# mbway/turbo

Measured on AMD Instinct MI355X. Metric: acquisition evals/sec (M candidates, N training) + GP-fit ms, higher is better.
Workload: dtype f32

## Files before the change

### turbo_amd/_lib.py

```python
import ctypes
import importlib.util
import os
import sys

import numpy as np

_HERE = os.path.dirname(os.path.abspath(__file__))

os.environ.setdefault("GPU_MAX_HW_QUEUES", "8")
LIB_PATH = os.environ.get("TGP_LIBRARY") or os.path.join(_HERE, "csrc", "libturbogp.so")

OK, NOT_PD, BAD_ARG, HIP_ERROR, NOT_FITTED, NO_MEMORY, NO_DEVICE = 0, 1, 2, 3, 4, 5, 6
DEVICE_HOST = -1
F64, F32, F32X3, F32H2 = 0, 1, 2, 3
KERNELS = {"rbf": 0, "matern12": 1, "matern32": 2, "matern52": 3}
ACQ_NONE, ACQ_UCB, ACQ_PI, ACQ_EI, ACQ_SIGMA, ACQ_MES = 0, 1, 2, 3, 4, 5
BUF_K, BUF_L, BUF_LINV, BUF_ALPHA = 0, 1, 2, 3
BATCH_KB, BATCH_CL = 0, 1

SYMBOLS = (
    "tgp_create", "tgp_destroy", "tgp_last_error", "tgp_version", "tgp_fit", "tgp_fit_grad", "tgp_loo", "tgp_fit_loo_grad", "tgp_fit_optimise", "tgp_fit_lbfgsb", "tgp_set_private_stream",
    "tgp_set_overlap", "tgp_tuning", "tgp_mt19937_uniform_columns", "tgp_set_candidates_mt19937", "tgp_stream_status", "tgp_workers_acquire", "tgp_workers_release",
    "tgp_fit_append", "tgp_export_state", "tgp_import_state", "tgp_export_factor_dev", "tgp_import_factor_dev", "tgp_debug_read",
    "tgp_set_candidates", "tgp_set_candidates_dev", "tgp_gen_candidates", "tgp_gen_candidates_lhs", "tgp_lhs_design",
# ... 829 lines not shown
        assert Xq.ndim == 2 and Xq.shape[1] == self.D, "points must be (m, %d)" % self.D
        val = np.empty(Xq.shape[0])
        grad = np.empty(Xq.shape)
        self._check(self.lib.tgp_acq_grad(self._h, _ptr(Xq), Xq.shape[0], acq, float(sf), float(incumbent),
                                          float(param), _ptr(val), _ptr(grad)))
        return val, grad

    def profile_enable(self, on=True):
        self._check(self.lib.tgp_profile_enable(self._h, 1 if on else 0))

    def profile_reset(self):
        self._check(self.lib.tgp_profile_reset(self._h))

    def profile_read(self):
        tl, kl = ctypes.c_int64(), ctypes.c_int64()
        tm, km, fm, sm = (ctypes.c_double() for _ in range(4))
        self._check(self.lib.tgp_profile_read(self._h, ctypes.byref(tl), ctypes.byref(tm),
                                              ctypes.byref(kl), ctypes.byref(km),
                                              ctypes.byref(fm), ctypes.byref(sm)))
        return dict(trmm_launches=tl.value, trmm_ms=tm.value, kstar_launches=kl.value,
                    kstar_ms=km.value, last_fit_ms=fm.value, last_sweep_ms=sm.value)

    def last_timings(self):
        v = np.zeros(12)
        self._check(self.lib.tgp_last_timings(self._h, _ptr(v), 12))
        return dict(fit_ms=v[0], sweep_ms=v[1], grad_kinv_ms=v[2], grad_pairwise_ms=v[3], grad_ard_ms=v[4],
                    trmm_flops=v[5], sweep_f64=int(v[6]), small_fit_phases_us=[float(x) for x in v[7:12]])

    def last_prune(self):
        v = np.zeros(19)
        self._check(self.lib.tgp_last_timings(self._h, _ptr(v), 19))
        return dict(state=int(v[12]), lb_set=int(v[13]), survivors=int(v[14]), screen=int(v[16]), screen_arith=int(v[18]))

    def sweep_geometry(self):
        ch, npad = ctypes.c_int64(), ctypes.c_int64()
        self._check(self.lib.tgp_sweep_geometry(self._h, ctypes.byref(ch), ctypes.byref(npad)))
        return ch.value, npad.value
```

### turbo_amd/csrc/sweep_pruned.hpp

```cpp
#pragma once

namespace tgp {

struct BoundArgs {
    const double *mupart, *abspart; long ldpart; int njs;
    long m;
    double err_scale;
    const double *err;
    const double *wcoef;
    const double *wadd;
    double y_mean, y_std;
    double sig_lo, sig_hi;
    int acq; double sf, incumbent, param, margin;
    double *ub;
};

__global__ __launch_bounds__(256) void prune_bound_kernel(BoundArgs b) {
    const long c = (long)blockIdx.x * 256 + threadIdx.x;
    if (c >= b.m) return;
    double mun = 0.0, s = 0.0;
    for (int j = 0; j < b.njs; ++j) {
        mun += b.mupart[(long)j * b.ldpart + c];
        if (!b.err || b.wcoef) s += b.abspart[(long)j * b.ldpart + c];
    }
    double e = b.err ? b.err[c] : b.err_scale * s;
    if (b.wcoef) e = screen_h2_error(e, b.wcoef[c], s, b.wadd[0]);
    const double mu = b.y_std * (b.sf > 0.0 ? mun + e : mun - e) + b.y_mean;
    const double a_lo = acq_value(b.acq, b.sf, b.incumbent, b.param, mu, b.sig_lo);
    const double a_hi = acq_value(b.acq, b.sf, b.incumbent, b.param, mu, b.sig_hi);
    double a = a_lo > a_hi ? a_lo : a_hi;
    double scale = fabs(a);
    if (b.acq == TGP_ACQ_UCB) scale += fabs(mu) + fabs(b.param) * b.sig_hi;
    a += b.margin * scale;
    b.ub[c] = (isnan(a_lo) || isnan(a_hi) || isnan(a)) ? INFINITY : a;
}

__global__ __launch_bounds__(256) void prune_pick_kernel(const double *__restrict__ ub, long m, long gs,
                                                         long long *__restrict__ pick) {
    __shared__ double sv[256];
    __shared__ long long si[256];
    const long g0 = (long)blockIdx.x * gs;
    const long g1 = g0 + gs < m ? g0 + gs : m;
    Best b;
    for (long c = g0 + threadIdx.x; c < g1; c += 256) {
        const double u = ub[c];
        if (u > b.v) { b.v = u; b.i = c; }
    }
    b = block_argmax<256>(b, sv, si);
    if (threadIdx.x == 0) pick[blockIdx.x] = b.i == IDX_NONE ? g0 : b.i;
}

template <typename T>
__global__ __launch_bounds__(256) void prune_gather_kernel(const T *__restrict__ Cs, int Dp, const long long *__restrict__ idx,
                                                           long n, long rows, T *__restrict__ out) {
    const long total = rows * Dp;
    for (long i = (long)blockIdx.x * 256 + threadIdx.x; i < total; i += (long)gridDim.x * 256) {
        const long r = i / Dp;
        const int d = (int)(i - r * Dp);
        out[i] = r < n ? Cs[idx[r] * Dp + d] : (T)0;
    }
}

struct SurvArgs {
    const double *ub; long m;
    const long long *pick; long gs;
    const double *lb; double margin;
    int *bcnt; const int *boff;
    long long *sidx;
    const long long *src;
};

__device__ __forceinline__ bool prune_survives(const SurvArgs &s, long c) {
    const double lb = s.lb[0];
    const double bar = isinf(lb) ? lb : lb - s.margin * fabs(lb);
    return c < s.m && s.ub[c] >= bar && (s.src || s.pick[c / s.gs] != c);
}

__global__ __launch_bounds__(256) void prune_count_kernel(SurvArgs s) {
    __shared__ int wsum[4];
    const long c = (long)blockIdx.x * 256 + threadIdx.x;
    const unsigned long long bal = __ballot(prune_survives(s, c));
    if ((threadIdx.x & 63) == 0) wsum[threadIdx.x >> 6] = __popcll(bal);
    __syncthreads();
    if (threadIdx.x == 0) s.bcnt[blockIdx.x] = wsum[0] + wsum[1] + wsum[2] + wsum[3];
}

__global__ __launch_bounds__(1024) void prune_scan_kernel(const int *__restrict__ bcnt, int nb, int *__restrict__ boff,
                                                          long long *__restrict__ total) {
    __shared__ int part[1024];
    const int per = (nb + 1023) / 1024;
    const int b0 = (int)threadIdx.x * per;
    const int b1 = b0 + per < nb ? b0 + per : nb;
    int s = 0;
    for (int b = b0; b < b1; ++b) s += bcnt[b];
    part[threadIdx.x] = s;
    __syncthreads();
    for (int o = 1; o < 1024; o <<= 1) {
        const int v = (int)threadIdx.x >= o ? part[threadIdx.x - o] : 0;
        __syncthreads();
        part[threadIdx.x] += v;
        __syncthreads();
    }
    int run = part[threadIdx.x] - s;
    for (int b = b0; b < b1; ++b) { boff[b] = run; run += bcnt[b]; }
    if (threadIdx.x == 1023) total[0] = part[1023];
}

__global__ __launch_bounds__(256) void prune_scatter_kernel(SurvArgs s) {
    __shared__ int wsum[4];
    const long c = (long)blockIdx.x * 256 + threadIdx.x;
    const bool keep = prune_survives(s, c);
    const unsigned long long bal = __ballot(keep);
    const int lane = threadIdx.x & 63, w = threadIdx.x >> 6;
    if (lane == 0) wsum[w] = __popcll(bal);
    __syncthreads();
    int off = s.boff[blockIdx.x];
    for (int k = 0; k < w; ++k) off += wsum[k];
    if (keep) s.sidx[off + __popcll(bal & ((1ull << lane) - 1ull))] = s.src ? s.src[c] : c;
}

struct PruneWs {
    double *ub; long long *pick, *sidx, *misc; int *bcnt, *boff; void *cs;
    double *err, *ub1; long long *sidx1; float *nx;
    double *wcoef; unsigned char *xh; float *nxp, *absa; long ncap;
};
static size_t al256(size_t b) { return (b + 255) & ~(size_t)255; }

struct Carver {
    char *base = nullptr;
    size_t off = 0;
    template <typename U>
    U *take(size_t count, bool wanted = true) {
        U *ptr = base ? reinterpret_cast<U *>(base + off) : nullptr;
        if (wanted) off += al256(count * sizeof(U));
        return ptr;
    }
};

template <typename T>
static void prune_carve(const Context &c, int64_t npick, int64_t rows_cap, bool screen, bool h2, Carver &k, PruneWs &w) {
    const size_t M = (size_t)c.M, nb = (size_t)((c.M + 255) / 256), Mpad = (size_t)c.ws_Mpad;
    w.ncap = (long)((c.N + SCR_T - 1) / SCR_T + 1) * SCR_T;
    const size_t ncap = (size_t)w.ncap, nch = (size_t)((c.Dp + SCR_DC - 1) / SCR_DC);
    w.ub = k.take<double>(M);
    w.pick = k.take<long long>((size_t)npick);
    w.sidx = k.take<long long>(M);
    w.misc = k.take<long long>(32);
    w.bcnt = k.take<int>(nb);
    w.boff = k.take<int>(nb);
    w.cs = k.take<T>((size_t)rows_cap * c.Dp);
    w.err = k.take<double>(Mpad, screen);
    w.ub1 = k.take<double>((size_t)rows_cap, screen);
    w.sidx1 = k.take<long long>(M, screen);
    w.nx = k.take<float>((size_t)c.Np, screen);
    w.wcoef = k.take<double>(Mpad, h2);
    w.xh = k.take<unsigned char>(nch * ncap * 128, h2);
    w.nxp = k.take<float>(ncap, h2);
    w.absa = k.take<float>(ncap, h2);
}

template <typename T>
static hipError_t prune_workspace(Context &c, int64_t npick, int64_t rows_cap, bool screen, bool h2, PruneWs &w) {
    Carver count;
    prune_carve<T>(c, npick, rows_cap, screen, h2, count, w);
    TGP_TRY(c.d_prune.reserve(count.off, [&] { return hipStreamSynchronize(c.stream); }));
    Carver k{c.d_prune};
    prune_carve<T>(c, npick, rows_cap, screen, h2, k, w);
    return hipSuccess;
}

template <typename T>
static TrmmVariant contract_variant(const SweepPlan<T> &p, int64_t rows, int ntm) {
    TrmmVariant v;
    v.kern = p.early.kern; v.lds = trmm_glds_lds_bytes(); v.tile_m = 128; v.tile_n = 128; v.threads = 256;
    if ((rows / 128) * ntm >= CONTRACT_MIN_WGS) return v;
    if ((rows / 64) * ntm >= CONTRACT_MIN_WGS) {
        v.kern = trmm_sumsq_glds_narrow_kernel<T, 64>; v.lds = trmm_narrow_lds_bytes<64>(); v.tile_n = 64;
    } else {
        v.kern = trmm_sumsq_glds_narrow_kernel<T, 32>; v.lds = trmm_narrow_lds_bytes<32>(); v.tile_n = 32;
    }
    return v;
}

template <typename T>
static hipError_t contract_rows(Context &c, const SweepPlan<T> &p, const T *cs, int64_t n, ProfCursor &cur) {
    for (int64_t off = 0; off < n; off += c.launch_rows) {
        const int64_t m = n - off < c.launch_rows ? n - off : c.launch_rows;
        const int64_t rows = pad128(m);
        const int ntile = (int)c.Np / 128;
        const int njs_s = grid_splits(rows / (16 * kstar_ar(sizeof(T))), GATHER_KS_MIN_WGS, ntile, ntile);
        const int njs_g = njs_s > p.njs ? njs_s : p.njs;
        TGP_TRY(launch_kstar<T>(c, Kstar::SlabNoMean, cs + off * c.Dp, rows, njs_g, c.d_Ks[0].get(), c.d_mupart + off,
                                (long)c.Np / 16, 1.f, cur.st));
        cur.seg(1);
        TGP_TRY(launch_trmm<T>(c, p, contract_variant<T>(p, rows, p.n128), 0, off, rows, 0, p.n128, 0, true, cur.st));
        cur.seg(0, (double)m * (double)c.N * (double)c.N);
    }
    return hipSuccess;
}

enum class PruneGo { NotEligible, GatedOff, Go };
template <typename T>
static PruneGo prune_eligible(const Context &c, const SweepPlan<T> &p, const SweepCall &call) {
    const int acq = call.acq;
    if (call.mu || call.sigma || call.acqv) return PruneGo::NotEligible;
    if (acq != TGP_ACQ_EI && acq != TGP_ACQ_PI && acq != TGP_ACQ_UCB) return PruneGo::NotEligible;
    if (c.dtype != TGP_F32 && c.dtype != TGP_F64) return PruneGo::NotEligible;
    if (!p.mean_in_trmm || tuning_sweep_prune_now() == 0) return PruneGo::NotEligible;
    if (!(c.M > tuning().prune_top)) return PruneGo::NotEligible;
    if (!((double)c.M * (double)c.N * (double)c.N >= tuning_prune_min_work_now())) return PruneGo::NotEligible;
    const double u = sizeof(T) == 4 ? 0x1p-24 : 0x1p-53;
    const bool gate = c.noise > 0.0 && c.noise / (c.constant + c.noise) >= tuning().prune_tau * u;
    return gate ? PruneGo::Go : PruneGo::GatedOff;
}

template <typename T>
struct PruneRun {
    Context &c;
    const SweepPlan<T> &p;
    const SweepCall &call;
    PruneWs w;
    BoundArgs b;
    const T *Cs, *Xs;
    T *cs;
    int64_t gs, npick, keep;
    bool screen, h2;
    ProfCursor cur;
};

template <typename T>
static hipError_t tight_bound(PruneRun<T> &r, const T *rowsrc, int64_t rows, int64_t m, double *ub) {
    Context &c = r.c;
    const int njs_b = grid_splits(rows / (16 * kstar_ar(sizeof(T))), BOUND_MIN_WGS, r.p.njs, r.p.njs);
    TGP_TRY(launch_kstar<T>(c, Kstar::Bound, rowsrc, rows, njs_b, c.d_part.get(), c.d_mupart, 0L, 1.f, c.stream));
    r.cur.seg(1);
    r.b.njs = njs_b; r.b.m = m; r.b.err = nullptr; r.b.wcoef = nullptr; r.b.ub = ub;
    hipLaunchKernelGGL(prune_bound_kernel, dim3((unsigned)((m + 255) / 256)), dim3(256), 0, c.stream, r.b);
    return hipGetLastError();
}

static hipError_t screen_h2_bound(PruneRun<float> &r, int64_t xb, int njs_s) {
    Context &c = r.c;
    const PruneWs &w = r.w;
    const int N = (int)c.N, Dp = (int)c.Dp;
    const ScreenH2Terms et = screen_h2_error_terms(c.constant, (int)c.D, N);
    ScreenH2Scal *scal = reinterpret_cast<ScreenH2Scal *>(w.misc + 8);
    static_assert(sizeof(ScreenH2Scal) <= 256 - 64, "the scalars live behind misc's first eight words");
    ScreenH2PrepArgs a{};
    a.Xs = r.Xs; a.alpha = c.d_alpha; a.N = N; a.Dp = Dp; a.nch = (Dp + SCR_DC - 1) / SCR_DC; a.ncap = w.ncap;
    a.P = et.P; a.Qc = et.Qc; a.Qw = et.Qw;
    a.Xh = w.xh; a.nxp = w.nxp; a.absa = w.absa; a.scal = scal;
    hipLaunchKernelGGL(screen_h2_prep_kernel, dim3((unsigned)((N + 255) / 256)), dim3(256), 0, c.stream, a);
    TGP_TRY(hipGetLastError());
    r.cur.restart();
    ScreenH2Args g{};
    g.Cs = r.Cs; g.Xh = w.xh; g.nxp = w.nxp; g.absa = w.absa; g.scal = scal;
    g.mupart = c.d_mupart; g.wpart = c.d_part; g.err = w.err; g.wcoef = w.wcoef; g.ldpart = c.ws_Mpad; g.ncap = w.ncap;
    g.Dp = Dp; g.constant = c.constant; g.dcoef = et.dcoef;
    hipLaunchKernelGGL(prune_screen_h2_kernel, dim3((unsigned)xb, (unsigned)njs_s), dim3(256), 0, c.stream, g);
    TGP_TRY(hipGetLastError());
// ... 11 lines not shown
    double *scal = reinterpret_cast<double *>(w.misc + 8);
    hipLaunchKernelGGL(screen_stats_kernel, dim3(1), dim3(1024), 0, c.stream, r.Xs, c.d_alpha, N, (int)c.Np, Dp, et.P, et.Q, w.nx, scal);
    TGP_TRY(hipGetLastError());
    r.cur.restart();
    ScreenArgs g{};
    g.Cs = r.Cs; g.Xs = r.Xs; g.alpha = c.d_alpha; g.nx = w.nx; g.scal = scal;
    g.mupart = c.d_mupart; g.err = w.err; g.ldpart = c.ws_Mpad;
    g.N = N; g.Np = (int)c.Np; g.Dp = Dp; g.constant = c.constant;
    hipLaunchKernelGGL(prune_screen_kernel, dim3((unsigned)xb, (unsigned)njs_s), dim3(256), 0, c.stream, g);
    TGP_TRY(hipGetLastError());
    r.cur.seg(2);
    c.prune_arith = 1;
    r.b.wcoef = nullptr;
    return hipSuccess;
}

template <typename T>
static hipError_t bound_all(PruneRun<T> &r) {
    Context &c = r.c;
    if (!r.screen) return tight_bound<T>(r, r.Cs, c.ws_Mpad, c.M, r.w.ub);
    if constexpr (sizeof(T) == 4) {
        const int64_t xb = c.ws_Mpad / SCR_T;
        const int njt = ((int)c.N + SCR_T - 1) / SCR_T;
        const int njs_s = grid_splits(xb, SCREEN_MIN_WGS, r.p.njs, njt < r.p.njs ? njt : r.p.njs);
        TGP_TRY(r.h2 ? screen_h2_bound(r, xb, njs_s) : screen_f32_bound(r, xb, njs_s));
        r.b.njs = njs_s; r.b.m = c.M; r.b.err = r.w.err; r.b.ub = r.w.ub;
        hipLaunchKernelGGL(prune_bound_kernel, dim3((unsigned)((c.M + 255) / 256)), dim3(256), 0, c.stream, r.b);
        return hipGetLastError();
    }
    return hipSuccess;
}

template <typename T>
static hipError_t gather_rows(PruneRun<T> &r, const long long *idx, int64_t n) {
    const int Dp = (int)r.c.Dp;
    const long total = (long)pad128(n) * Dp;
    const long blocks = (total + 255) / 256 < 8192 ? (total + 255) / 256 : 8192;
    hipLaunchKernelGGL(prune_gather_kernel<T>, dim3((unsigned)blocks), dim3(256), 0, r.c.stream, r.Cs, Dp, idx, (long)n,
                       (long)pad128(n), r.cs);
    return hipGetLastError();
}

template <typename T>
static hipError_t finalize_rows(PruneRun<T> &r, const long long *idx, int64_t n, int64_t blk0) {
    FinArgs f = fin_args<T>(r.c, r.p, r.call);
    f.base_pairs = r.p.nunits;
    f.njs = 1;
    f.off = blk0 * FIN_BLOCK; f.m = n;
    f.gidx = idx;
    hipLaunchKernelGGL(finalize_kernel, dim3((unsigned)((n + FIN_BLOCK - 1) / FIN_BLOCK)), dim3(FIN_BLOCK), 0, r.c.stream, f);
    return hipGetLastError();
}

template <typename T>
static hipError_t lb_set(PruneRun<T> &r, int64_t &nblk) {
    Context &c = r.c;
    hipLaunchKernelGGL(prune_pick_kernel, dim3((unsigned)r.npick), dim3(256), 0, c.stream, r.w.ub, (long)c.M, (long)r.gs, r.w.pick);
    TGP_TRY(hipGetLastError());
    TGP_TRY(gather_rows(r, r.w.pick, r.npick));
    TGP_TRY(contract_rows<T>(c, r.p, r.cs, r.npick, r.cur));
    TGP_TRY(finalize_rows(r, r.w.pick, r.npick, 0));
    nblk = (r.npick + FIN_BLOCK - 1) / FIN_BLOCK;
    return launch_argmax(c, c.stream, (long)nblk, nullptr, nullptr, Bell{nullptr, 0, nullptr});
}

template <typename T>
static hipError_t survivors(PruneRun<T> &r, const double *ub, int64_t m, const long long *src, long long *out, long long &n) {
    Context &c = r.c;
    const PruneWs &w = r.w;
    hipStream_t st = c.stream;
    const int64_t nb = (m + 255) / 256;
    SurvArgs s{ub, (long)m, w.pick, (long)r.gs, c.d_best, r.b.margin, w.bcnt, w.boff, out, src};
    hipLaunchKernelGGL(prune_count_kernel, dim3((unsigned)nb), dim3(256), 0, st, s);
    TGP_TRY(hipGetLastError());
    hipLaunchKernelGGL(prune_scan_kernel, dim3(1), dim3(1024), 0, st, w.bcnt, (int)nb, w.boff, w.misc);
    TGP_TRY(hipGetLastError());
    hipLaunchKernelGGL(prune_scatter_kernel, dim3((unsigned)nb), dim3(256), 0, st, s);
    TGP_TRY(hipGetLastError());
    TGP_TRY(hipMemcpyAsync(&n, w.misc, sizeof(long long), hipMemcpyDeviceToHost, st));
    return hipStreamSynchronize(st);
}

template <typename T>
static hipError_t narrow_after_screen(PruneRun<T> &r, long long &nsurv, const long long *&sidx) {
    Context &c = r.c;
    const PruneWs &w = r.w;
    if (nsurv > r.keep) {
        r.cur.restart();
        TGP_TRY(tight_bound<T>(r, r.Cs, c.ws_Mpad, c.M, w.ub));
        TGP_TRY(survivors(r, w.ub, c.M, nullptr, w.sidx, nsurv));
    } else if (nsurv > tuning_prune_direct_now()) {
        TGP_TRY(gather_rows(r, w.sidx, nsurv));
        r.cur.restart();
        TGP_TRY(tight_bound<T>(r, r.cs, pad128(nsurv), nsurv, w.ub1));
        const long long n0 = nsurv;
        TGP_TRY(survivors(r, w.ub1, n0, w.sidx, w.sidx1, nsurv));
        sidx = w.sidx1;
    }
    r.cur.restart();
    return hipSuccess;
}

template <typename T>
static hipError_t contract_survivors_and_pick(PruneRun<T> &r, const long long *sidx, int64_t nsurv, int64_t nblk_lb) {
    int64_t nblk = 0;
    if (nsurv > 0) {
        TGP_TRY(gather_rows(r, sidx, nsurv));
        TGP_TRY(contract_rows<T>(r.c, r.p, r.cs, nsurv, r.cur));
        TGP_TRY(finalize_rows(r, sidx, nsurv, nblk_lb));
        nblk = (nsurv + FIN_BLOCK - 1) / FIN_BLOCK;
    }
    return launch_argmax(r.c, r.c.stream, (long)(nblk_lb + nblk), r.call.winner, r.call.res, Bell{nullptr, 0, nullptr});
}

static BoundArgs bound_args(const Context &c, const SweepCall &call, double margin) {
    BoundArgs b{};
    b.mupart = c.d_mupart; b.abspart = c.d_part; b.ldpart = c.ws_Mpad;
    b.err_scale = 4.0 * (double)((int)c.N + 8) * 0x1p-53;
    b.y_mean = c.y_mean; b.y_std = c.y_std;
    b.sig_lo = sqrt((0.99 * c.noise) * (c.y_std * c.y_std));
    b.sig_hi = sqrt((c.constant + c.noise) * (c.y_std * c.y_std));
    b.acq = call.acq; b.sf = call.sf; b.incumbent = call.incumbent; b.param = call.param; b.margin = margin;
    return b;
}

template <typename T>
static hipError_t sweep_pruned(Context &c, const SweepPlan<T> &p, const SweepCall &call, bool front_usable, bool &done) {
    done = false;
    const Tuning &tu = tuning();
    const int64_t M = c.M;
    const int64_t top = tu.prune_top < 1 ? 1 : tu.prune_top;
    const int64_t gs = (M + top - 1) / top, npick = (M + gs - 1) / gs;
    const double frac = tuning_prune_frac_now();
    const int64_t keep = frac < 0.0 ? -1 : (frac >= 1.0 ? M : (int64_t)(frac * (double)M));
    const int64_t rows_cap = pad128(npick > keep ? npick : keep);
    const bool screen = sizeof(T) == 4 && c.kernel == TGP_RBF && c.D <= SCR_MAXD && tuning_prune_screen_now() != 0;
    const bool h2 = screen && tuning_screen_arith_now() == 2 && c.D >= SCRH_MIN_D;
    PruneRun<T> r{c, p, call, PruneWs{}, BoundArgs{}, reinterpret_cast<const T *>(c.d_Cs.get()), train_points<T>(c), nullptr,
                  gs, npick, keep, screen, h2, ProfCursor{c, c.stream, -1}};
    TGP_TRY(prune_workspace<T>(c, npick, rows_cap, screen, h2, r.w));
    TGP_TRY(lds_opt_in(c, p.early.kern, p.early.lds));
    r.cs = reinterpret_cast<T *>(r.w.cs);
    c.prune_screen = -1;
    c.prune_arith = 0;
    if (!front_usable) TGP_TRY(issue_prep<T>(c, c.stream));
    r.cur.restart();
    r.b = bound_args(c, call, tu.prune_margin);

    TGP_TRY(bound_all(r));
    int64_t nblk_lb = 0;
    TGP_TRY(lb_set(r, nblk_lb));
    long long nsurv = 0;
    const long long *sidx = r.w.sidx;
    TGP_TRY(survivors(r, r.w.ub, M, nullptr, r.w.sidx, nsurv));
    c.prune_lbset = npick;
    if (screen) {
        c.prune_screen = nsurv;
        TGP_TRY(narrow_after_screen(r, nsurv, sidx));
    }
    c.prune_surv = nsurv;
    if (nsurv > keep) {
        c.prune_state = 1;
        return hipMemsetAsync(c.d_besti + 1, 0, sizeof(long long), c.stream);
    }
    TGP_TRY(contract_survivors_and_pick(r, sidx, nsurv, nblk_lb));
    c.prune_state = 0;
    done = true;
    return hipSuccess;
}

}
```

### turbo_amd/csrc/tgp_api.hip

```cpp
#include <hip/hip_runtime.h>
#include <math.h>
#include <stdlib.h>
#include <string.h>

#include <algorithm>
#include <atomic>
#include <chrono>
#include <condition_variable>
#include <functional>
#include <mutex>
#include <new>
#include <string>
#include <system_error>
#include <thread>
#include <vector>

#include "host_backend.hpp"
#include "host_lbfgsb.hpp"
#include "host_slice.hpp"
#include "tgp_internal.hpp"

using namespace tgp;

struct tgp_handle_s {
// ... 1392 lines not shown
static int acq_check_args(Context &c, const char *fn, const char *own, int acq, int acq_max, double sf) {
    if (!c.fitted) return fail(c, TGP_NOT_FITTED, std::string(fn) + ": no fitted model");
    if (own) return fail(c, TGP_BAD_ARG, std::string(fn) + ": " + own);
    return acq_check(c, fn, acq, acq_max, sf);
}
static int box_check(Context &c, const char *fn, const double *lo, const double *hi) {
    for (int64_t d = 0; d < c.D; ++d)
        if (!(lo[d] <= hi[d])) return fail(c, TGP_BAD_ARG, std::string(fn) + ": need lo <= hi in every dimension");
    return TGP_OK;
}

static int winner_mark(Context &c, const SweepCall &s) {
    if (!s.winner || s.acq == TGP_ACQ_NONE) return TGP_OK;
    API_HIP(c.ev_winner.create(hipEventDisableTiming), "hipEventCreate");
    API_HIP(hipEventRecord(c.ev_winner, c.stream), "hipEventRecord");
    c.winner_recorded = true;
    return TGP_OK;
}

static int run_sweep(Context &c, const SweepCall &call, CallClock &clk) {
    SweepCall s = call;
    if (s.acq == TGP_ACQ_MES) s.mes = MesArgs{c.d_mes, c.mes_S, c.noise * (c.y_std * c.y_std)};
    const SweepPath path = sweep_path(c, c.M);
    int rc = path == SweepPath::General ? ensure_workspace(c) : ensure_small_workspace(c);
    if (rc != TGP_OK) return rc;
    const bool front = path == SweepPath::General && s.may_use_front && c.pre.gen == c.fit_gen && c.pre.cand == c.d_cand &&
                       c.pre.M == c.M && c.pre.Mpad == c.ws_Mpad && c.pre.launch_rows == c.launch_rows && c.pre.chunk == c.chunk;
    c.pre.front = false;
    c.last_sweep_f64 = path != SweepPath::General || c.dtype == TGP_F64;
    c.prune_state = -1;
    c.prune_lbset = c.prune_surv = 0;
    c.prune_screen = -1;
    c.prune_arith = 0;
    if ((rc = call_begin(c, clk)) != TGP_OK) return rc;
    hipError_t le;
    if (path == SweepPath::OneLaunch) {
        le = launch_mid_sweep(c, s);
    } else if (path == SweepPath::OneWorkgroup) {
        le = launch_small_sweep(c, s);
        if (le == hipSuccess) le = launch_argmax_final(c, s);
    } else {
        le = launch_sweep(c, s, front);
    }
    if (le != hipSuccess) return hip_fail(c, le, "launch_sweep");
    return winner_mark(c, s);
}

struct SweepRecord { double bv = 0.0; long long bi[2] = {0, 0}; };
static int sweep_queue_return(Context &c, bool zc, int acq, SweepRecord &r, CallClock *clk, double *mu, double *sigma, double *acq_out) {
    if (!zc) {
        if (acq != TGP_ACQ_NONE) API_HIP(hipMemcpyAsync(&r.bv, c.d_best, sizeof(double), hipMemcpyDeviceToHost, c.stream), "D2H best");
        API_HIP(hipMemcpyAsync(r.bi, c.d_besti, 2 * sizeof(long long), hipMemcpyDeviceToHost, c.stream), "D2H besti");
        API_HIP(hipMemsetAsync(c.d_besti, 0, 4 * sizeof(long long), c.stream), "memset counters");
    }
    if (clk) API_MEM(call_stop(c, *clk));
    const size_t bytes = (size_t)c.M * sizeof(double);
    if (mu) API_HIP(hipMemcpyAsync(mu, c.d_mu, bytes, hipMemcpyDeviceToHost, c.stream), "D2H mu");
    if (sigma) API_HIP(hipMemcpyAsync(sigma, c.d_sigma, bytes, hipMemcpyDeviceToHost, c.stream), "D2H sigma");
    if (acq_out) API_HIP(hipMemcpyAsync(acq_out, c.d_acq, bytes, hipMemcpyDeviceToHost, c.stream), "D2H acq");
    return TGP_OK;
}
static void sweep_read_record(Context &c, bool zc, int acq, SweepRecord &r, double *best_val, int64_t *best_idx, int64_t *n_clamped) {
    if (c.profiling) prof_collect(c);
    if (zc) { r.bv = c.h_pin_out[0]; r.bi[0] = (long long)c.h_pin_out[1]; r.bi[1] = (long long)c.h_pin_out[2]; }
    if (acq != TGP_ACQ_NONE) {
        if (best_val) *best_val = r.bv;
// ... 1336 lines not shown

int tgp_profile_read(tgp_handle h, int64_t *trmm_launches, double *trmm_ms, int64_t *kstar_launches,
                     double *kstar_ms, double *last_fit_ms, double *last_sweep_ms) try {
    if (!h) return TGP_BAD_ARG;
    if (h->host) {
        if (trmm_launches) *trmm_launches = 0;
        if (trmm_ms) *trmm_ms = 0.0;
        if (kstar_launches) *kstar_launches = 0;
        if (kstar_ms) *kstar_ms = 0.0;
        if (last_fit_ms) *last_fit_ms = h->host->last_fit_ms;
        if (last_sweep_ms) *last_sweep_ms = h->host->last_sweep_ms;
        return TGP_OK;
    }
    Context &c = h->c;
    prof_collect(c);
    if (trmm_launches) *trmm_launches = c.trmm_launches;
    if (trmm_ms) *trmm_ms = c.trmm_ms;
    if (kstar_launches) *kstar_launches = c.kstar_launches;
    if (kstar_ms) *kstar_ms = c.kstar_ms;
    if (last_fit_ms) *last_fit_ms = c.last_fit_ms;
    if (last_sweep_ms) *last_sweep_ms = c.last_sweep_ms;
    return TGP_OK;
} TGP_CATCH

int tgp_last_timings(tgp_handle h, double *out, int64_t n) try {
    if (!h) return TGP_BAD_ARG;
    if (h->host) {
        if (!out || n < 1) { h->host->err = "tgp_last_timings: need out and n >= 1"; return TGP_BAD_ARG; }
        for (int64_t i = 0; i < n; ++i) out[i] = i == 0 ? h->host->last_fit_ms : (i == 1 ? h->host->last_sweep_ms : (i == 6 ? 1.0 : (i == 12 || i == 16 ? -1.0 : 0.0)));
        return TGP_OK;
    }
    Context &c = h->c;
    if (!out || n < 1) return fail(c, TGP_BAD_ARG, "tgp_last_timings: need out and n >= 1");
    double v[21] = {c.last_fit_ms, c.last_sweep_ms, c.last_grad_ms[0], c.last_grad_ms[1], c.last_grad_ms[2], c.trmm_flops,
                    (double)c.last_sweep_f64, 0.0, 0.0, 0.0, 0.0, 0.0, (double)c.prune_state, (double)c.prune_lbset,
                    (double)c.prune_surv, c.last_cov_ms, (double)c.prune_screen, c.screen_ms, (double)c.prune_arith, c.last_loo_ms, c.last_kg_ms};
    if (c.h_bell && c.h_bell[1]) {
        const unsigned long long t0 = c.h_bell[1];
        const int src[5] = {3, 4, 5, 6, 2};
        for (int k = 0; k < 5; ++k) v[7 + k] = c.h_bell[src[k]] >= t0 ? (double)(c.h_bell[src[k]] - t0) * 1e-2 : 0.0;
    }
    for (int64_t i = 0; i < n; ++i) out[i] = i < 21 ? v[i] : 0.0;
    return TGP_OK;
} TGP_CATCH

int tgp_sweep_geometry(tgp_handle h, int64_t *chunk, int64_t *n_padded) try {
    if (!h) return TGP_BAD_ARG;
    if (h->host) { if (chunk) *chunk = 16; if (n_padded) *n_padded = h->host->N; return TGP_OK; }
    if (chunk) *chunk = h->c.chunk;
    if (n_padded) *n_padded = h->c.Np;
    return TGP_OK;
} TGP_CATCH

}
```

### turbo_amd/csrc/tgp_internal.hpp

```cpp
#pragma once
#include <hip/hip_runtime.h>
#include <stdint.h>

#include <string>
#include <type_traits>
#include <utility>
#include <vector>

#include "../../include/turbogp.h"
#include "dev_mem.hpp"
#include "doorbell.hpp"
#include "lds_opt_in.hpp"
#include "mes_math.hpp"
#include "tuning.hpp"

namespace tgp {


constexpr int NB = 64;
constexpr int NPAD = 256;
constexpr int SW_BM = 128;
constexpr int SW_BN = 128;
constexpr int KS_JS = 8;
constexpr int FIN_BLOCK = 256;
// ... 125 lines not shown
    Dev<int> d_flag;
    bool grad_staged = false;
    bool grad_timed = true;
    double last_loo_ms = 0.0;
    double last_cov_ms = 0.0;
    long fit_gen = 0;
    float linv16_sb = 0.f;
    bool imported = false;
    int64_t import_rows = 0;
    int64_t fit_gen_src = -1;

    bool small = false;
    int64_t linv_extent = 0;
    Pin<double> h_pin_in{hipHostMallocMapped | hipHostMallocCoherent};
    Pin<double> h_pin_out{hipHostMallocMapped | hipHostMallocCoherent};
    Pin<double> h_pin_cand{hipHostMallocMapped};
    Pin<uint32_t> h_mt_words{hipHostMallocDefault, false};
    Ev ev_mt[2];
    Pin<unsigned long long> h_bell{hipHostMallocMapped | hipHostMallocCoherent};
    unsigned long long bell_seq = 0;
    Dev<unsigned> d_ticket;
    Dev<double> d_sfg;

    const double *d_cand = nullptr;
    Dev<double> d_cand_owned;
    int64_t M = 0;

    int64_t chunk = 0;
    int64_t launch_rows = 0;
    int prune_state = -1;
    int64_t prune_lbset = 0, prune_surv = 0;
    int64_t prune_screen = -1;
    int prune_arith = 0;
    double screen_ms = 0.0;
    Dev<double> d_bval;
    Dev<long long> d_bidx;
    double *d_winner = nullptr;
    int64_t winner_offset = 0;
    Ev ev_winner;
    bool winner_recorded = false;
    Dev<double> d_best;
    Dev<long long> d_besti;

    bool profiling = false;
    std::vector<Ev> ev_pool;
    size_t ev_used = 0;
    std::vector<ProfSeg> segs;
    int64_t trmm_launches = 0, kstar_launches = 0;
    double trmm_ms = 0.0, kstar_ms = 0.0;
    double trmm_flops = 0.0;
    double last_fit_ms = 0.0, last_sweep_ms = 0.0;
    int last_sweep_f64 = -1;
};

hipStream_t private_fit_begin(int device, bool may_borrow);
void private_fit_end(int device, bool held);
hipError_t launch_fit(Context &c, const double *staged_in, double *res_host, bool zero_linv = true, unsigned long long *start_stamp = nullptr);
hipError_t launch_ring(Context &c, const Bell &bell);
hipError_t device_streams(int device, hipStream_t *main, hipStream_t *bg, hipStream_t *pre = nullptr);
void device_streams_release(int device);
void device_stream_status(int device, int *bg_ok, int *pre_ok);
hipError_t launch_lml_grad(Context &c, bool ard, double *gout, bool timed = true);
hipError_t launch_kinv_product(Context &c);
hipError_t launch_pair_sums(Context &c, bool ard, const double *loo_b, double *gout, bool timed);
constexpr int LOO_ROWS = 256;
constexpr double LOO_LOG_2PI = 1.8378770664093453;
// ... 191 lines not shown
```

### turbo_amd/csrc/tuning.hpp

```cpp
#pragma once
#include <stdio.h>
#include <stdlib.h>
#include <string.h>

#include <string>

namespace tgp {

#define TGP_TUNING_TABLE(X)                                                                                                      \
                                                        \
    X(INT, chunk, "TGP_CHUNK", 0, "candidates per slab group (multiple of 1024; 0 = about 256 MiB of slab) [per call]")          \
    X(DBL, slab_gb, "TGP_SLAB_GB", 1.0, "GiB of cross-kernel slab per launch pair (groups of TGP_CHUNK inside it)")              \
    X(STR, tile, "TGP_TILE", "", "contraction tile: 128 | 256x128 | 256x256 (default: by launch size)")                         \
    X(INT, nbuf, "TGP_NBUF", 0, "LDS k-tile buffers of the 256x128 contraction: 2 | 3 (default: 3 for f64, 2 for f32)")          \
    X(STR, trmm, "TGP_TRMM", "", "reg = the register-staged contraction template instead of the direct-to-LDS kernels (A/B)")    \
    X(INT, bk, "TGP_BK", 0, "k-tile of the contraction (f32: 16 | 32 | 64, f64: 8 | 16 | 32); other than 128 bytes = template")  \
    X(INT, mfma16, "TGP_MFMA16", 0, "1 = v_mfma_f32_16x16x4 fragments in the 128-tile f32 contraction")                         \
    X(INT, ks_js, "TGP_KS_JS", 0, "splits of the training points over the cross-kernel grid (0 = up to 8)")                       \
    X(INT, sweep_zc, "TGP_SWEEP_ZC", 1, "0 = the sweep's result record by D2H copies + memset instead of mapped host memory")    \
    X(INT, mean_in_trmm, "TGP_MEAN", 1, "1 = posterior mean K*.alpha accumulated inside the contraction's full-k row tiles (f64 / f32); 0 = in the cross-kernel (round 4)") \
    X(INT, overlap, "TGP_OVERLAP", 2, "sweep started inside tgp_fit for the resident batch: 0 = never, 1 = scaling + first cross-kernel, 2 = + contraction row tiles whose rows of Linv are final") \
    X(INT, pre_tiles, "TGP_PRE_TILES", -1, "128-row tiles of the first launch pair contracted inside the fit in mode 2 (-1 = a quarter of the rows)") \
    X(INT, pre_cus, "TGP_PRE_CUS", -1, "CUs of the third stream, which carries the sweep's front inside a fit (-1 = three quarters of the device, 0 = unmasked)") \
    X(INT, pre_cu0, "TGP_PRE_CU0", 0, "first CU of that mask")                                                                 \
    X(INT, pre_lds_kb, "TGP_PRE_LDS_KB", 81, "KiB of LDS requested per workgroup of the early contraction (64 = two per CU, 81 = one)") \
    X(INT, sweep_prune, "TGP_SWEEP_PRUNE", 1, "1 = an arg-max-only EI / PI / UCB sweep (f32 / f64, N > 256) contracts only the candidates whose acquisition bound can still win (sweep_pruned); 0 = every candidate [per call]") \
    X(INT, prune_top, "TGP_PRUNE_TOP", 256, "candidates of the pruned sweep's lb set (the best bound of each of this many groups): its best exact value is the bar") \
    X(DBL, prune_frac, "TGP_PRUNE_FRAC", 0.25, "the pruned sweep runs the full schedule when more than this share of the batch survives (< 0: always) [per call]") \
    X(DBL, prune_min_work, "TGP_PRUNE_MIN_WORK", 1e11, "the pruned sweep runs only when M * N^2 (the full contraction's multiply-adds) reaches this: below, its fixed cost is more than it saves [per call]") \
    X(DBL, prune_tau, "TGP_PRUNE_TAU", 2e4, "the pruned sweep needs s^2 / (c + s^2) >= this * the contraction's unit roundoff (no skipped candidate can clamp)") \
    X(INT, prune_screen, "TGP_PRUNE_SCREEN", 1, "1 = the pruned sweep of an f32 RBF handle screens every candidate on the matrix cores first (prune_screen.hpp) and runs its tight bound pass only on the screen's survivors; 0 = the tight bound pass over all candidates [per call]") \
    X(STR, screen_arith, "TGP_SCREEN_ARITH", "h2", "arithmetic of that screen: h2 = two fp16 planes per operand on v_mfma_f32_32x32x16_f16 and a k-weighted error (prune_screen_h2.hpp; D >= 15, else f32), f32 = prune_screen.hpp's kernel and closed form; the A/B switch [per call]") \
    X(INT, prune_direct, "TGP_PRUNE_DIRECT", 1024, "screen survivors up to this many are contracted as they are; more (up to TGP_PRUNE_FRAC of the batch) go through the tight bound pass first [per call]") \
    X(DBL, prune_margin, "TGP_PRUNE_MARGIN", 1e-6, "relative slack of the pruned sweep's bounds against the bar (rounding of the acquisition formulas)") \
    X(INT, mid, "TGP_MID", 1, "0 = 128 < N <= 256 down the general sweep instead of the one-launch kernel")                      \
    X(INT, mid_maxm, "TGP_MID_MAXM", 0, "largest batch that takes the one-launch sweep for 256 < N <= 512 (0 = never) [per call]") \
    X(INT, small, "TGP_SMALL", 1, "0 = N <= 128 down the blocked path instead of the one-workgroup kernels")                     \
                                                                         \
    X(INT, ob, "TGP_OB", 0, "outer block of the Cholesky (multiple of 256; 0 = by size: all of Np <= 1024, else 256 / 512 / 1024)") \
    X(INT, panel, "TGP_PANEL", 5, "diagonal-block factorisation: 5 = variant D (LDS block, MFMA), 3 / 38 = C, 4 / 8 = B, 0 = round 1") \
    X(INT, panel_la, "TGP_PANEL_LA", 1, "0 = pivot factored in the panel launch instead of beside the previous update")          \
    X(INT, panel_fuse, "TGP_PANEL_FUSE", 1, "0 = two launches per panel instead of fused_panel_kernel")                          \
    X(INT, panel_fuse_tiles, "TGP_PANEL_FUSE_TILES", 384, "fused panel launches for outer blocks whose first update has at most this many tiles") \
    X(STR, inner, "TGP_INNER", "", "gemm64 = the in-block rank-64 update on the generic template")                               \
    X(STR, gemm64, "TGP_GEMM64", "", "reg = the f64 64x64 NT products on the register-staged template (A/B, bit-identical)")     \
    X(INT, trail64, "TGP_TRAIL64", 8192, "trailing updates of up to this many rows on 64x64 tiles (beyond: 128-tile kernel)")    \
    X(INT, merge64, "TGP_MERGE64", 2048, "inverse merges with a leading block up to this on 64x64 tiles")                        \
    X(INT, kinv64, "TGP_KINV64", 4096, "K^-1 = U U^T of the LML gradient on 64x64 tiles up to this Np")                          \
    X(INT, bginv, "TGP_BGINV", 1, "0 = the inverse level by level after the factorisation instead of behind the panel chain")   \
    X(INT, level64_fused, "TGP_LEVEL64_FUSED", 1, "0 = the 64 -> 128 level of the inverse as three launches (two products + transpose) instead of one") \
    X(INT, bginv_max, "TGP_BGINV_MAX", 9216, "largest Np whose inverse runs behind the chain")                                   \
    X(INT, bg_lease, "TGP_BG_LEASE", 1, "0 = a fit on a private stream never borrows the background stream (its inverse always in line)") \
    X(INT, bg_cus, "TGP_BG_CUS", -1, "CUs of the background stream (-1 = three quarters of the device, 0 = unmasked)")           \
    X(INT, bg_probe, "TGP_BG_PROBE", 1, "0 = skip the probe that the stream pair really overlaps")                               \
    X(INT, linv_zero, "TGP_LINV_ZERO", 0, "1 = every fit zero-fills Linv (default: only when it may hold stale rows)")           \
    X(STR, stamp_file, "TGP_STAMP_FILE", "", "debug: the panel chain's in-kernel time stamps are dumped to this file")           \
                                                                                             \
    X(INT, hyper_wgs, "TGP_HYPER_WGS", 0, "1 = one workgroup per start in the one-launch hyper-parameter fit (default: 3 for 64 < N <= 128)") \
    X(INT, hyper_threads, "TGP_HYPER_THREADS", 0, "host threads of tgp_fit_lbfgsb (0 = by size: 4 to N = 1536, 3 to 8192, 1 beyond)") \
                                                                                      \
    X(INT, poll_us, "TGP_POLL_US", 50000, "microseconds a short call (small fit, fit + gradient, acquisition gradient) spins on its doorbell before it synchronises the stream instead (0 = never poll: events + hipStreamSynchronize as in round 5)") \
    X(INT, small_live, "TGP_SMALL_LIVE", 1, "0 = the N <= 128 fit factors the identity padding of its 64-blocks too and fetches the targets a second time (round 5's body; same bytes)") \
    X(INT, small_fused, "TGP_SMALL_FUSED", 1, "0 = N <= 128 fit + LML gradient as two launches (round 5) instead of one")          \
    X(INT, small_query, "TGP_SMALL_QUERY", 1, "0 = tgp_acq_grad for N <= 128 down the general kernels instead of one workgroup per point") \
    X(INT, query_mfma, "TGP_QUERY_MFMA", 1, "0 = the two triangular products of tgp_acq_grad above N = 128 on the wave-per-row / split-column kernels instead of v_mfma_f64_16x16x4 (A/B; same values to rounding)") \
                                                                                                    \
// ... 48 lines not shown
#undef TGP_TD_STR
        return out;
    }
};

inline const Tuning &tuning() {
    static const Tuning t;
    return t;
}

inline int runtime_hw_queues_env() { const char *v = getenv("GPU_MAX_HW_QUEUES"); return v ? atoi(v) : 0; }

inline const Tuning &tuning_defaults() {
    static const Tuning t(false);
    return t;
}
namespace tuning_env {
#define TGP_TE(kind, f, env, d, doc) constexpr const char *f = env;
TGP_TUNING_TABLE(TGP_TE)
#undef TGP_TE
}
inline int now_int(const char *env, int dflt) { const char *v = getenv(env); return v ? atoi(v) : dflt; }
inline double now_dbl(const char *env, double dflt) { const char *v = getenv(env); return v ? atof(v) : dflt; }
inline std::string now_str(const char *env, const std::string &dflt) { const char *v = getenv(env); return v ? v : dflt; }
#define TGP_NOW(kind, f) now_##kind(tuning_env::f, tuning_defaults().f)
inline int tuning_chunk_now() { return TGP_NOW(int, chunk); }
inline int tuning_mid_maxm_now() { return TGP_NOW(int, mid_maxm); }
inline int tuning_sweep_prune_now() { return TGP_NOW(int, sweep_prune); }
inline double tuning_prune_frac_now() { return TGP_NOW(dbl, prune_frac); }
inline int tuning_prune_screen_now() { return TGP_NOW(int, prune_screen); }
inline int tuning_screen_arith_now() { return TGP_NOW(str, screen_arith) == "f32" ? 1 : 2; }
inline int tuning_prune_direct_now() { return TGP_NOW(int, prune_direct); }
inline double tuning_prune_min_work_now() { return TGP_NOW(dbl, prune_min_work); }
#undef TGP_NOW

}
```

Before: 84.14 million.

## Speculatively contract group runner-ups in the pruned sweep to skip survivor round

When the previous sweep kept few survivors, the pruned acquisition sweep now takes the top-4 bounds per group, picks the best runner-ups (up to a cap), and contracts them together with the lower-bound set in one round. If every survivor is already among the contracted rows, the survivors' contraction round and its extra launches are skipped and the argmax runs directly. This costs extra work in the lb-set round (a top-4 pick kernel, a ranking kernel, more gathered rows, and an atomic leftover count). If speculation misses, it falls back to the old path after doing that extra work.

```diff
diff --git a/turbo_amd/_lib.py b/turbo_amd/_lib.py
--- a/turbo_amd/_lib.py
+++ b/turbo_amd/_lib.py
@@ -885,6 +885,11 @@
         self._check(self.lib.tgp_last_timings(self._h, _ptr(v), 19))
         return dict(state=int(v[12]), lb_set=int(v[13]), survivors=int(v[14]), screen=int(v[16]), screen_arith=int(v[18]))
 
+    def last_prune_spec(self):
+        v = np.zeros(22)
+        self._check(self.lib.tgp_last_timings(self._h, _ptr(v), 22))
+        return int(v[21])
+
     def sweep_geometry(self):
         ch, npad = ctypes.c_int64(), ctypes.c_int64()
         self._check(self.lib.tgp_sweep_geometry(self._h, ctypes.byref(ch), ctypes.byref(npad)))
diff --git a/turbo_amd/csrc/sweep_pruned.hpp b/turbo_amd/csrc/sweep_pruned.hpp
--- a/turbo_amd/csrc/sweep_pruned.hpp
+++ b/turbo_amd/csrc/sweep_pruned.hpp
@@ -50,14 +50,82 @@
     if (threadIdx.x == 0) pick[blockIdx.x] = b.i == IDX_NONE ? g0 : b.i;
 }
 
+__global__ __launch_bounds__(256) void prune_pick4_kernel(const double *__restrict__ ub, long m, long gs, long long *__restrict__ pick,
+                                                          long long *__restrict__ runner) {
+    __shared__ double sv[256];
+    __shared__ long long si[256];
+    const long g0 = (long)blockIdx.x * gs;
+    const long g1 = g0 + gs < m ? g0 + gs : m;
+    double v[4] = {-INFINITY, -INFINITY, -INFINITY, -INFINITY};
+    long long ix[4] = {IDX_NONE, IDX_NONE, IDX_NONE, IDX_NONE};
+    for (long c = g0 + threadIdx.x; c < g1; c += 256) {
+        const double u = ub[c];
+        if (better(u, c, v[3], ix[3])) {
+            v[3] = u; ix[3] = c;
+#pragma unroll
+            for (int k = 3; k > 0; --k)
+                if (better(v[k], ix[k], v[k - 1], ix[k - 1])) {
+                    const double tv = v[k]; v[k] = v[k - 1]; v[k - 1] = tv;
+                    const long long ti = ix[k]; ix[k] = ix[k - 1]; ix[k - 1] = ti;
+                }
+        }
+    }
+#pragma unroll
+    for (int round = 0; round < 4; ++round) {
+        Best b;
+        b.v = v[0]; b.i = ix[0];
+        b = block_argmax<256>(b, sv, si);
+        __syncthreads();
+        if (b.i != IDX_NONE && b.i == ix[0]) {
+            v[0] = v[1]; v[1] = v[2]; v[2] = v[3]; v[3] = -INFINITY;
+            ix[0] = ix[1]; ix[1] = ix[2]; ix[2] = ix[3]; ix[3] = IDX_NONE;
+        }
+        if (threadIdx.x == 0) {
+            if (round == 0) pick[blockIdx.x] = b.i == IDX_NONE ? g0 : b.i;
+            else runner[3 * (long)blockIdx.x + round - 1] = b.i;
+        }
+    }
+}
+
+constexpr int SPEC_MAXR = 3072;
+__global__ __launch_bounds__(256) void prune_extras_kernel(const double *__restrict__ ub, const long long *__restrict__ runner, int R,
+                                                           int cap, long long nx, long long *__restrict__ extras,
+                                                           int *__restrict__ sel, long long *__restrict__ words) {
+    __shared__ double sv[SPEC_MAXR];
+    __shared__ long long si[SPEC_MAXR];
+    for (int k = threadIdx.x; k < R; k += 256) {
+        const long long i = runner[k];
+        si[k] = i;
+        sv[k] = i == IDX_NONE ? -INFINITY : ub[i];
+    }
+    __syncthreads();
+    if (blockIdx.x == 0 && threadIdx.x == 0) { words[1] = 0; words[2] = nx; }
+    const int lane = threadIdx.x & 63;
+    const int k = (int)blockIdx.x * 4 + (threadIdx.x >> 6);
+    if (k >= R) return;
+    const double vk = sv[k];
+    const long long ik = si[k];
+    int rank = 0;
+    for (int j0 = 0; j0 < R; j0 += 64) {
+        const int j = j0 + lane;
+        rank += __popcll(__ballot(j < R && better(sv[j], si[j], vk, ik)));
+    }
+    if (lane == 0) {
+        const int take = ik != IDX_NONE && rank < cap;
+        sel[k] = take;
+        if (take) extras[rank] = ik;
+    }
+}
+
 template <typename T>
 __global__ __launch_bounds__(256) void prune_gather_kernel(const T *__restrict__ Cs, int Dp, const long long *__restrict__ idx,
-                                                           long n, long rows, T *__restrict__ out) {
+                                                           long n, const long long *__restrict__ idx1, long n1, long rows,
+                                                           T *__restrict__ out) {
     const long total = rows * Dp;
     for (long i = (long)blockIdx.x * 256 + threadIdx.x; i < total; i += (long)gridDim.x * 256) {
         const long r = i / Dp;
         const int d = (int)(i - r * Dp);
-        out[i] = r < n ? Cs[idx[r] * Dp + d] : (T)0;
+        out[i] = r < n ? Cs[idx[r] * Dp + d] : (r < n + n1 ? Cs[idx1[r - n] * Dp + d] : (T)0);
     }
 }
 
@@ -68,6 +136,9 @@
     int *bcnt; const int *boff;
     long long *sidx;
     const long long *src;
+    const long long *runner;
+    const int *sel;
+    int *leftover;
 };
 
 __device__ __forceinline__ bool prune_survives(const SurvArgs &s, long c) {
@@ -116,13 +187,23 @@
     __syncthreads();
     int off = s.boff[blockIdx.x];
     for (int k = 0; k < w; ++k) off += wsum[k];
-    if (keep) s.sidx[off + __popcll(bal & ((1ull << lane) - 1ull))] = s.src ? s.src[c] : c;
+    if (keep) {
+        const long long gc = s.src ? s.src[c] : c;
+        s.sidx[off + __popcll(bal & ((1ull << lane) - 1ull))] = gc;
+        if (s.runner) {
+            const long g3 = 3 * (long)(gc / s.gs);
+            bool found = false;
+            for (int k = 0; k < 3; ++k) found = found || (s.runner[g3 + k] == gc && s.sel[g3 + k] != 0);
+            if (!found) atomicAdd(s.leftover, 1);
+        }
+    }
 }
 
 struct PruneWs {
     double *ub; long long *pick, *sidx, *misc; int *bcnt, *boff; void *cs;
     double *err, *ub1; long long *sidx1; float *nx;
     double *wcoef; unsigned char *xh; float *nxp, *absa; long ncap;
+    long long *runner, *extras; int *sel;
 };
 static size_t al256(size_t b) { return (b + 255) & ~(size_t)255; }
 
@@ -138,7 +219,7 @@
 };
 
 template <typename T>
-static void prune_carve(const Context &c, int64_t npick, int64_t rows_cap, bool screen, bool h2, Carver &k, PruneWs &w) {
+static void prune_carve(const Context &c, int64_t npick, int64_t rows_cap, bool screen, bool h2, bool spec, Carver &k, PruneWs &w) {
     const size_t M = (size_t)c.M, nb = (size_t)((c.M + 255) / 256), Mpad = (size_t)c.ws_Mpad;
     w.ncap = (long)((c.N + SCR_T - 1) / SCR_T + 1) * SCR_T;
     const size_t ncap = (size_t)w.ncap, nch = (size_t)((c.Dp + SCR_DC - 1) / SCR_DC);
@@ -157,15 +238,18 @@
     w.xh = k.take<unsigned char>(nch * ncap * 128, h2);
     w.nxp = k.take<float>(ncap, h2);
     w.absa = k.take<float>(ncap, h2);
-}
-
-template <typename T>
-static hipError_t prune_workspace(Context &c, int64_t npick, int64_t rows_cap, bool screen, bool h2, PruneWs &w) {
+    w.runner = k.take<long long>(3 * (size_t)npick, spec);
+    w.extras = k.take<long long>(3 * (size_t)npick, spec);
+    w.sel = k.take<int>(3 * (size_t)npick, spec);
+}
+
+template <typename T>
+static hipError_t prune_workspace(Context &c, int64_t npick, int64_t rows_cap, bool screen, bool h2, bool spec, PruneWs &w) {
     Carver count;
-    prune_carve<T>(c, npick, rows_cap, screen, h2, count, w);
+    prune_carve<T>(c, npick, rows_cap, screen, h2, spec, count, w);
     TGP_TRY(c.d_prune.reserve(count.off, [&] { return hipStreamSynchronize(c.stream); }));
     Carver k{c.d_prune};
-    prune_carve<T>(c, npick, rows_cap, screen, h2, k, w);
+    prune_carve<T>(c, npick, rows_cap, screen, h2, spec, k, w);
     return hipSuccess;
 }
 
@@ -226,6 +310,7 @@
     int64_t gs, npick, keep;
     bool screen, h2;
     ProfCursor cur;
+    int64_t nx = 0;
 };
 
 template <typename T>
@@ -303,18 +388,19 @@
 }
 
 template <typename T>
-static hipError_t gather_rows(PruneRun<T> &r, const long long *idx, int64_t n) {
+static hipError_t gather_rows(PruneRun<T> &r, const long long *idx, int64_t n, const long long *idx1 = nullptr, int64_t n1 = 0) {
     const int Dp = (int)r.c.Dp;
-    const long total = (long)pad128(n) * Dp;
+    const long total = (long)pad128(n + n1) * Dp;
     const long blocks = (total + 255) / 256 < 8192 ? (total + 255) / 256 : 8192;
-    hipLaunchKernelGGL(prune_gather_kernel<T>, dim3((unsigned)blocks), dim3(256), 0, r.c.stream, r.Cs, Dp, idx, (long)n,
-                       (long)pad128(n), r.cs);
+    hipLaunchKernelGGL(prune_gather_kernel<T>, dim3((unsigned)blocks), dim3(256), 0, r.c.stream, r.Cs, Dp, idx, (long)n, idx1,
+                       (long)n1, (long)pad128(n + n1), r.cs);
     return hipGetLastError();
 }
 
 template <typename T>
-static hipError_t finalize_rows(PruneRun<T> &r, const long long *idx, int64_t n, int64_t blk0) {
+static hipError_t finalize_rows(PruneRun<T> &r, const long long *idx, int64_t n, int64_t blk0, int64_t col0 = 0) {
     FinArgs f = fin_args<T>(r.c, r.p, r.call);
+    f.part += col0; f.mupart += col0;
     f.base_pairs = r.p.nunits;
     f.njs = 1;
     f.off = blk0 * FIN_BLOCK; f.m = n;
@@ -336,20 +422,48 @@
 }
 
 template <typename T>
-static hipError_t survivors(PruneRun<T> &r, const double *ub, int64_t m, const long long *src, long long *out, long long &n) {
+static hipError_t lb_set_with_extras(PruneRun<T> &r, int64_t &nblk, int64_t &nblk_x) {
+    Context &c = r.c;
+    const PruneWs &w = r.w;
+    hipLaunchKernelGGL(prune_pick4_kernel, dim3((unsigned)r.npick), dim3(256), 0, c.stream, w.ub, (long)c.M, (long)r.gs, w.pick, w.runner);
+    TGP_TRY(hipGetLastError());
+    const int R = (int)(3 * r.npick);
+    hipLaunchKernelGGL(prune_extras_kernel, dim3((unsigned)((R + 3) / 4)), dim3(256), 0, c.stream, w.ub, w.runner, R, (int)r.nx,
+                       (long long)r.nx, w.extras, w.sel, w.misc);
+    TGP_TRY(hipGetLastError());
+    TGP_TRY(gather_rows(r, w.pick, r.npick, w.extras, r.nx));
+    TGP_TRY(contract_rows<T>(c, r.p, r.cs, r.npick + r.nx, r.cur));
+    TGP_TRY(finalize_rows(r, w.pick, r.npick, 0));
+    nblk = (r.npick + FIN_BLOCK - 1) / FIN_BLOCK;
+    TGP_TRY(finalize_rows(r, w.extras, r.nx, nblk, r.npick));
+    nblk_x = (r.nx + FIN_BLOCK - 1) / FIN_BLOCK;
+    return launch_argmax(c, c.stream, (long)nblk, nullptr, nullptr, Bell{nullptr, 0, nullptr});
+}
+
+template <typename T>
+static hipError_t survivors(PruneRun<T> &r, const double *ub, int64_t m, const long long *src, long long *out, long long &n,
+                            long long *leftover = nullptr) {
     Context &c = r.c;
     const PruneWs &w = r.w;
     hipStream_t st = c.stream;
     const int64_t nb = (m + 255) / 256;
-    SurvArgs s{ub, (long)m, w.pick, (long)r.gs, c.d_best, r.b.margin, w.bcnt, w.boff, out, src};
+    SurvArgs s{ub, (long)m, w.pick, (long)r.gs, c.d_best, r.b.margin, w.bcnt, w.boff, out, src, nullptr, nullptr, nullptr};
+    if (leftover) { s.runner = w.runner; s.sel = w.sel; s.leftover = reinterpret_cast<int *>(w.misc + 1); }
     hipLaunchKernelGGL(prune_count_kernel, dim3((unsigned)nb), dim3(256), 0, st, s);
     TGP_TRY(hipGetLastError());
     hipLaunchKernelGGL(prune_scan_kernel, dim3(1), dim3(1024), 0, st, w.bcnt, (int)nb, w.boff, w.misc);
     TGP_TRY(hipGetLastError());
     hipLaunchKernelGGL(prune_scatter_kernel, dim3((unsigned)nb), dim3(256), 0, st, s);
     TGP_TRY(hipGetLastError());
-    TGP_TRY(hipMemcpyAsync(&n, w.misc, sizeof(long long), hipMemcpyDeviceToHost, st));
-    return hipStreamSynchronize(st);
+    if (!leftover) {
+        TGP_TRY(hipMemcpyAsync(&n, w.misc, sizeof(long long), hipMemcpyDeviceToHost, st));
+        return hipStreamSynchronize(st);
+    }
+    long long back[2] = {0, 0};
+    TGP_TRY(hipMemcpyAsync(back, w.misc, sizeof back, hipMemcpyDeviceToHost, st));
+    TGP_TRY(hipStreamSynchronize(st));
+    n = back[0]; *leftover = back[1];
+    return hipSuccess;
 }
 
 template <typename T>
@@ -404,27 +518,52 @@
     const int64_t gs = (M + top - 1) / top, npick = (M + gs - 1) / gs;
     const double frac = tuning_prune_frac_now();
     const int64_t keep = frac < 0.0 ? -1 : (frac >= 1.0 ? M : (int64_t)(frac * (double)M));
-    const int64_t rows_cap = pad128(npick > keep ? npick : keep);
+    const int spec_mode = tuning_prune_spec_now();
+    const int64_t cap = tuning_prune_spec_cap_now();
+    const int64_t last = M - (npick - 1) * gs;
+    const int64_t nrunner = (npick - 1) * (gs - 1 < 3 ? gs - 1 : 3) + (last - 1 < 3 ? last - 1 : 3);
+    const int64_t nx_max = spec_mode != 0 && cap > 0 && 3 * npick <= SPEC_MAXR ? (cap < nrunner ? cap : nrunner) : 0;
+    const bool spec = nx_max > 0 && (spec_mode >= 2 || (c.prune_hist >= 1 && c.prune_hist <= cap));
+    const int64_t rows_cap = pad128(npick + nx_max > keep ? npick + nx_max : keep);
     const bool screen = sizeof(T) == 4 && c.kernel == TGP_RBF && c.D <= SCR_MAXD && tuning_prune_screen_now() != 0;
     const bool h2 = screen && tuning_screen_arith_now() == 2 && c.D >= SCRH_MIN_D;
     PruneRun<T> r{c, p, call, PruneWs{}, BoundArgs{}, reinterpret_cast<const T *>(c.d_Cs.get()), train_points<T>(c), nullptr,
                   gs, npick, keep, screen, h2, ProfCursor{c, c.stream, -1}};
-    TGP_TRY(prune_workspace<T>(c, npick, rows_cap, screen, h2, r.w));
+    TGP_TRY(prune_workspace<T>(c, npick, rows_cap, screen, h2, nx_max > 0, r.w));
     TGP_TRY(lds_opt_in(c, p.early.kern, p.early.lds));
     r.cs = reinterpret_cast<T *>(r.w.cs);
     c.prune_screen = -1;
     c.prune_arith = 0;
+    c.prune_hist = -1;
     if (!front_usable) TGP_TRY(issue_prep<T>(c, c.stream));
     r.cur.restart();
     r.b = bound_args(c, call, tu.prune_margin);
+    r.nx = spec ? nx_max : 0;
 
     TGP_TRY(bound_all(r));
-    int64_t nblk_lb = 0;
-    TGP_TRY(lb_set(r, nblk_lb));
-    long long nsurv = 0;
+    int64_t nblk_lb = 0, nblk_x = 0;
+    long long nsurv = 0, leftover = 0;
     const long long *sidx = r.w.sidx;
-    TGP_TRY(survivors(r, r.w.ub, M, nullptr, r.w.sidx, nsurv));
+    if (spec) {
+        TGP_TRY(lb_set_with_extras(r, nblk_lb, nblk_x));
+        TGP_TRY(survivors(r, r.w.ub, M, nullptr, r.w.sidx, nsurv, &leftover));
+    } else {
+        TGP_TRY(lb_set(r, nblk_lb));
+        TGP_TRY(survivors(r, r.w.ub, M, nullptr, r.w.sidx, nsurv));
+    }
     c.prune_lbset = npick;
+    const long long nsurv0 = nsurv;
+    if (spec && leftover == 0 && nsurv <= r.nx && nsurv <= keep && (!screen || nsurv <= tuning_prune_direct_now())) {
+        if (screen) c.prune_screen = nsurv;
+        c.prune_surv = nsurv;
+        c.prune_spec = 1;
+        TGP_TRY(launch_argmax(c, c.stream, (long)(nblk_lb + nblk_x), call.winner, call.res, Bell{nullptr, 0, nullptr}));
+        c.prune_state = 0;
+        c.prune_hist = nsurv0;
+        done = true;
+        return hipSuccess;
+    }
+    if (spec) c.prune_spec = 2;
     if (screen) {
         c.prune_screen = nsurv;
         TGP_TRY(narrow_after_screen(r, nsurv, sidx));
@@ -436,6 +575,7 @@
     }
     TGP_TRY(contract_survivors_and_pick(r, sidx, nsurv, nblk_lb));
     c.prune_state = 0;
+    c.prune_hist = nsurv0;
     done = true;
     return hipSuccess;
 }
diff --git a/turbo_amd/csrc/tgp_api.hip b/turbo_amd/csrc/tgp_api.hip
--- a/turbo_amd/csrc/tgp_api.hip
+++ b/turbo_amd/csrc/tgp_api.hip
@@ -1448,6 +1448,7 @@
     c.prune_lbset = c.prune_surv = 0;
     c.prune_screen = -1;
     c.prune_arith = 0;
+    c.prune_spec = 0;
     if ((rc = call_begin(c, clk)) != TGP_OK) return rc;
     hipError_t le;
     if (path == SweepPath::OneLaunch) {
@@ -2850,15 +2851,16 @@
     }
     Context &c = h->c;
     if (!out || n < 1) return fail(c, TGP_BAD_ARG, "tgp_last_timings: need out and n >= 1");
-    double v[21] = {c.last_fit_ms, c.last_sweep_ms, c.last_grad_ms[0], c.last_grad_ms[1], c.last_grad_ms[2], c.trmm_flops,
+    double v[22] = {c.last_fit_ms, c.last_sweep_ms, c.last_grad_ms[0], c.last_grad_ms[1], c.last_grad_ms[2], c.trmm_flops,
                     (double)c.last_sweep_f64, 0.0, 0.0, 0.0, 0.0, 0.0, (double)c.prune_state, (double)c.prune_lbset,
-                    (double)c.prune_surv, c.last_cov_ms, (double)c.prune_screen, c.screen_ms, (double)c.prune_arith, c.last_loo_ms, c.last_kg_ms};
+                    (double)c.prune_surv, c.last_cov_ms, (double)c.prune_screen, c.screen_ms, (double)c.prune_arith, c.last_loo_ms, c.last_kg_ms,
+                    (double)c.prune_spec};
     if (c.h_bell && c.h_bell[1]) {
         const unsigned long long t0 = c.h_bell[1];
         const int src[5] = {3, 4, 5, 6, 2};
         for (int k = 0; k < 5; ++k) v[7 + k] = c.h_bell[src[k]] >= t0 ? (double)(c.h_bell[src[k]] - t0) * 1e-2 : 0.0;
     }
-    for (int64_t i = 0; i < n; ++i) out[i] = i < 21 ? v[i] : 0.0;
+    for (int64_t i = 0; i < n; ++i) out[i] = i < 22 ? v[i] : 0.0;
     return TGP_OK;
 } TGP_CATCH
 
diff --git a/turbo_amd/csrc/tgp_internal.hpp b/turbo_amd/csrc/tgp_internal.hpp
--- a/turbo_amd/csrc/tgp_internal.hpp
+++ b/turbo_amd/csrc/tgp_internal.hpp
@@ -181,6 +181,8 @@
     int64_t prune_lbset = 0, prune_surv = 0;
     int64_t prune_screen = -1;
     int prune_arith = 0;
+    int prune_spec = 0;
+    int64_t prune_hist = -1;
     double screen_ms = 0.0;
     Dev<double> d_bval;
     Dev<long long> d_bidx;
diff --git a/turbo_amd/csrc/tuning.hpp b/turbo_amd/csrc/tuning.hpp
--- a/turbo_amd/csrc/tuning.hpp
+++ b/turbo_amd/csrc/tuning.hpp
@@ -32,6 +32,8 @@
     X(INT, prune_screen, "TGP_PRUNE_SCREEN", 1, "1 = the pruned sweep of an f32 RBF handle screens every candidate on the matrix cores first (prune_screen.hpp) and runs its tight bound pass only on the screen's survivors; 0 = the tight bound pass over all candidates [per call]") \
     X(STR, screen_arith, "TGP_SCREEN_ARITH", "h2", "arithmetic of that screen: h2 = two fp16 planes per operand on v_mfma_f32_32x32x16_f16 and a k-weighted error (prune_screen_h2.hpp; D >= 15, else f32), f32 = prune_screen.hpp's kernel and closed form; the A/B switch [per call]") \
     X(INT, prune_direct, "TGP_PRUNE_DIRECT", 1024, "screen survivors up to this many are contracted as they are; more (up to TGP_PRUNE_FRAC of the batch) go through the tight bound pass first [per call]") \
+    X(INT, prune_spec, "TGP_PRUNE_SPEC", 1, "the pruned sweep contracts its groups' runner-ups in the lb set's round and skips the survivors' round when they cover every survivor: 0 = never, 1 = after a sweep that kept 1 .. TGP_PRUNE_SPEC_CAP survivors, 2 = always [per call]") \
+    X(INT, prune_spec_cap, "TGP_PRUNE_SPEC_CAP", 128, "runner-ups taken into that round at most (the largest bounds among the second to fourth of each group) [per call]") \
     X(DBL, prune_margin, "TGP_PRUNE_MARGIN", 1e-6, "relative slack of the pruned sweep's bounds against the bar (rounding of the acquisition formulas)") \
     X(INT, mid, "TGP_MID", 1, "0 = 128 < N <= 256 down the general sweep instead of the one-launch kernel")                      \
     X(INT, mid_maxm, "TGP_MID_MAXM", 0, "largest batch that takes the one-launch sweep for 256 < N <= 512 (0 = never) [per call]") \
@@ -146,6 +148,8 @@
 inline int tuning_screen_arith_now() { return TGP_NOW(str, screen_arith) == "f32" ? 1 : 2; }
 inline int tuning_prune_direct_now() { return TGP_NOW(int, prune_direct); }
 inline double tuning_prune_min_work_now() { return TGP_NOW(dbl, prune_min_work); }
+inline int tuning_prune_spec_now() { return TGP_NOW(int, prune_spec); }
+inline int tuning_prune_spec_cap_now() { return TGP_NOW(int, prune_spec_cap); }
 #undef TGP_NOW
 
 }
```

Result: faster. 87.62 million, median of 6 (+4.1%).
